# Princic-1837592/julia-raytracer

Hardware: AMD Instinct MI355X
Metric: Mrays/s + wall-clock render time, cornellbox 1280×720×256spp (higher is better)
Workload: dtype f32; 1 GPU; cornellbox path 1280x720x256spp; scene=cornellbox, sampler=path, width=1280, height=720, spp=256, bounces=8, batch=256, traversal=near, traversal_requested=auto, bvh=middle, parallelism=1 tile groups x 1 sample ranges + RCCL reduce

## Files before the change

### julia-raytracer_amd/csrc/jt_kernels.h

```cpp
#pragma once

#include <hip/hip_runtime.h>

#include <algorithm>

#include "jt_bsdf.h"
#include "jt_device.h"
#include "jt_push.h"

#ifndef JT_STAMPS
#define JT_STAMPS 0
#endif
#ifndef JT_NODE_REPEAT_NONE
#define JT_NODE_REPEAT_NONE 4
#endif
#ifndef JT_NODE_REPEAT
#define JT_NODE_REPEAT 3
#endif
#ifndef JT_FIRST_POP_NONE
#define JT_FIRST_POP_NONE 1
#endif
#ifndef JT_FIRST_POP
#define JT_FIRST_POP 2
#endif
// ... 218 lines not shown
    p.scattering = V3(m.scattering[0], m.scattering[1], m.scattering[2]) * xyz(scattering_tex);
    p.scanisotropy = m.scanisotropy;
    p.trdepth = m.trdepth;
    if ((F & FT_VOL) && (mtype == M_REFRACTIVE || mtype == M_VOLUMETRIC || mtype == M_SUBSURFACE)) {
        p.density = V3(-jl_log(jl_clamp(p.color.x, 0.0001f, 1.0f)) / p.trdepth,
                       -jl_log(jl_clamp(p.color.y, 0.0001f, 1.0f)) / p.trdepth,
                       -jl_log(jl_clamp(p.color.z, 0.0001f, 1.0f)) / p.trdepth);
    } else {
        p.density = V3(0, 0, 0);
    }
    if (mtype == M_MATTE || mtype == M_GLTFPBR || mtype == M_GLOSSY) roughness = jl_clamp(roughness, min_roughness, 1.0f);
    else if (mtype == M_VOLUMETRIC) roughness = 0.0f;
    else if (roughness < min_roughness) roughness = 0.0f;
    p.roughness = roughness;
}

template <int F>
__device__ __forceinline__ v3 eval_environment(const DScene& S, v3 direction) {
    v3 emission = V3(0, 0, 0);
    if (!(F & FT_ENV)) return emission;
    for (int k = 0; k < S.nenvs; k++) {
        const DEnv& env = S.envs[k];
        v3 wl = transform_direction(frame_from(env.inv), direction);
        v2 tc = V2(jl_atan2(wl.z, wl.x) / (2.0f * pif), jl_acos(jl_clamp(wl.y, -1.0f, 1.0f)) / pif);
        if (tc.x < 0.0f) tc.x = tc.x + 1.0f;
        v4 t = eval_texture(S, env.tex, tc, false);
        emission = emission + V3(env.emission[0], env.emission[1], env.emission[2]) * xyz(t);
    }
    return emission;
}

constexpr int BLOCK = 256;
constexpr unsigned T_TLAS = 0u, T_INST = 1u, T_BLAS = 2u;
constexpr unsigned IDX_MASK = (1u << 24) - 1;
constexpr unsigned SNAP_NONE = 63u << 24;

struct Hit {
    int inst, elem;
    float u, v, t;
    bool hit;
};
struct Counters {
    unsigned nodes, instances, prims, shades;
};

struct Trav {
    v3 wo, wd, wdinv;
    v3 lo, ld, ldinv;
    float tmax;
    int sp;
    int low;
    int inst_space;
    int negmask;
    int cur_inst, cur_kind;
    int prim, nprim;
    int h_inst, h_elem;
    float h_u, h_v;
    int nh;
    unsigned nxt;
};

#ifndef JT_BAND_STRIP
#define JT_BAND_STRIP 16
#endif
#ifndef JT_TIE_RERUN
#define JT_TIE_RERUN 1
#endif
constexpr int TIE_SEEN = 1 << 8, REF_RERUN = 1 << 9, NH_COUNT = 63;
__device__ __forceinline__ int query_flip(const DScene& S, const Trav& T) { return (T.nh & REF_RERUN) ? 0 : S.order_flip; }
__device__ __forceinline__ void hit_count(Trav& T, float t) {
    T.nh = (T.nh + ((T.nh & NH_COUNT) < NH_COUNT ? 1 : 0)) | (JT_TIE_RERUN && t == T.tmax ? TIE_SEEN : 0);
}

__device__ __forceinline__ int neg_mask(v3 d, int flip) {
    return ((d.x < 0 ? 1 : 0) | (d.y < 0 ? 2 : 0) | (d.z < 0 ? 4 : 0)) ^ flip;
}

__device__ __forceinline__ void world_ray(const DScene& S, Trav& T) {
    T.lo = T.wo;
    T.ld = T.wd;
    T.ldinv = T.wdinv;
    T.negmask = neg_mask(T.wd, query_flip(S, T));
    T.inst_space = 0;
}

__device__ __forceinline__ Hit query_hit(const Trav& T) {
    return Hit{T.h_inst, T.h_elem, T.h_u, T.h_v, T.tmax, T.h_inst >= 0};
}

__device__ __forceinline__ bool query_busy(const Trav& T) { return T.sp > 0 || T.nprim > 0; }
template <bool WIDE>
__device__ __forceinline__ bool wants_node(const Trav& T) {
    return T.nprim == 0 && (T.sp > 0 || (WIDE && T.nxt != W_EMPTY));
}
template <bool WIDE>
__device__ __forceinline__ bool query_done(const Trav& T) {
    return (T.sp | T.nprim) == 0 && (!WIDE || T.nxt == W_EMPTY);
}

__device__ __forceinline__ void query_begin(const DScene& S, Trav& T, v3 o, v3 d, unsigned root, int* stack, int rerun = 0) {
    T.wo = o;
    T.wd = d;
    T.wdinv = V3(jl_rcp(d.x), jl_rcp(d.y), jl_rcp(d.z));
    T.lo = o;
    T.ld = d;
    T.ldinv = T.wdinv;
    T.tmax = __builtin_inff();
    T.nh = rerun;
    T.h_inst = -1;
    T.h_elem = -1;
    T.h_u = 0;
    T.h_v = 0;
    T.nprim = 0;
    T.prim = 0;
    T.cur_inst = -1;
    T.cur_kind = KIND_TRI;
    T.inst_space = 0;
    T.negmask = neg_mask(d, rerun ? 0 : S.order_flip);
    stack[0] = (int)root;
    T.sp = 1;
    T.low = 0;
    T.nxt = W_EMPTY;
}
__device__ __forceinline__ void query_begin_wide(const DScene& S, Trav& T, v3 o, v3 d, unsigned root_word, int rerun = 0) {
    T.wo = o;
    T.wd = d;
    T.wdinv = V3(jl_rcp(d.x), jl_rcp(d.y), jl_rcp(d.z));
    T.lo = o;
    T.ld = d;
    T.ldinv = T.wdinv;
    T.tmax = __builtin_inff();
    T.nh = rerun;
    T.h_inst = -1;
    T.h_elem = -1;
    T.h_u = 0;
    T.h_v = 0;
    T.nprim = 0;
    T.prim = 0;
    T.cur_inst = -1;
    T.cur_kind = KIND_TRI;
    T.inst_space = 0;
    T.negmask = neg_mask(d, rerun ? 0 : S.order_flip);
    T.sp = 0;
    T.low = 0;
    T.nxt = root_word;
}
constexpr unsigned WROOT_SCENE = 0u;
__device__ __forceinline__ unsigned wroot_instance(int inst) { return W_LEAF | W_INST | (unsigned)inst; }
template <bool WIDE>
__device__ __forceinline__ void query_start(const DScene& S, Trav& T, v3 o, v3 d, int inst, int* stack, int rerun = 0) {
    if (WIDE) query_begin_wide(S, T, o, d, inst < 0 ? WROOT_SCENE : wroot_instance(inst), rerun);
    else query_begin(S, T, o, d, inst < 0 ? ((T_TLAS << 30) | SNAP_NONE) : ((T_INST << 30) | SNAP_NONE | (unsigned)inst), stack, rerun);
}
constexpr int INST_LEAF_ROOT = 1 << 30;
template <bool WIDE>
__device__ __forceinline__ bool rerun_tie(const DScene& S, Trav& T, v3 o, v3 d, int inst, int* stack) {
    if (!JT_TIE_RERUN || (T.nh & (TIE_SEEN | REF_RERUN)) != TIE_SEEN || S.order_flip == 0) return false;
    if (inst >= 0 && (S.inst_blas[inst].w & INST_LEAF_ROOT)) return false;
    query_start<WIDE>(S, T, o, d, inst, stack, REF_RERUN);
    return true;
}

template <int F>
__device__ __forceinline__ void tri_pair(const DScene& S, Trav& T, int k) {
    const float4* r = S.prims + 5 * (T.prim + (k >> 1));
    const float4 r0 = r[0], r1 = r[1], r2 = r[2], r3 = r[3], r4 = r[4];
    const PrimHit p1 = intersect_triangle_pre(T.lo, T.ld, ray_eps, V3(r0.x, r0.z, r1.x), V3(r1.z, r2.x, r2.z),
                                              V3(r3.x, r3.z, r4.x));
    const PrimHit p2 = intersect_triangle_pre(T.lo, T.ld, ray_eps, V3(r0.y, r0.w, r1.y), V3(r1.w, r2.y, r2.w),
                                              V3(r3.y, r3.w, r4.y));
    if (tri_hit_before(p1, T.tmax)) {
        hit_count(T, p1.t);
        T.h_inst = T.cur_inst;
        T.h_elem = __float_as_int(r4.z);
        T.h_u = p1.u;
        T.h_v = p1.v;
        T.tmax = p1.t;
    }
    if (T.nprim >= k + 2 && tri_hit_before(p2, T.tmax)) {
        hit_count(T, p2.t);
        T.h_inst = T.cur_inst;
        T.h_elem = __float_as_int(r4.w);
        T.h_u = p2.u;
        T.h_v = p2.v;
        T.tmax = p2.t;
    }
}
template <int COUNT, int F>
__device__ __forceinline__ void prim_step(const DScene& S, Trav& T, Counters& cnt) {
    if (!(F & FT_QUAD) || T.cur_kind == KIND_TRI) {
        tri_pair<F>(S, T, 0);
        const bool more = T.nprim > 2;
        if (__builtin_amdgcn_ballot_w64(more)) {
            if (more) tri_pair<F>(S, T, 2);
        }
        const int n = T.nprim < 4 ? T.nprim : 4;
        if (COUNT) cnt.prims += n;
        T.prim += 2;
        T.nprim -= n;
        return;
    }
    if (COUNT) cnt.prims++;
    const float4* r = S.prims + 4 * T.prim;
    const float4 a = r[0], b = r[1], c = r[2], d = r[3];
    const PrimHit p = intersect_quad(T.lo, T.ld, ray_eps, T.tmax, xyz(a), xyz(b), xyz(c), xyz(d), d.w != 0.0f);
    if (p.hit) {
        hit_count(T, p.t);
        T.h_inst = T.cur_inst;
        T.h_elem = __float_as_int(a.w);
        T.h_u = p.u;
        T.h_v = p.v;
        T.tmax = p.t;
    }
    T.prim += 1;
    T.nprim -= 1;
}

template <int RING, bool OVF>
__device__ __forceinline__ void st_push(const DScene& S, Trav& T, int* stack, int pixel, unsigned e) {
    if (OVF) {
        if (T.sp - T.low == S.ring) {
            S.ovf[(size_t)pixel * S.ovf_stride + T.low] = stack[(T.low & (S.ring - 1)) * BLOCK];
            T.low += 1;
        }
        stack[(T.sp & (S.ring - 1)) * BLOCK] = (int)e;
    } else {
        stack[T.sp * BLOCK] = (int)e;
    }
    T.sp += 1;
}
template <int RING, bool OVF>
__device__ __forceinline__ unsigned st_pop(const DScene& S, Trav& T, const int* stack, int pixel) {
    T.sp -= 1;
    if (OVF) {
        const unsigned r = (unsigned)__hip_atomic_load(stack + (T.sp & (S.ring - 1)) * BLOCK, __ATOMIC_RELAXED,
                                                       __HIP_MEMORY_SCOPE_WORKGROUP);
        if (T.sp < T.low) {
            T.low = T.sp;
            return (unsigned)S.ovf[(size_t)pixel * S.ovf_stride + T.sp];
        }
        return r;
    }
    return (unsigned)stack[T.sp * BLOCK];
}

template <int RING, bool OVF, int COUNT, bool NCACHE, int F>
__device__ __forceinline__ void node_step(const DScene& S, Trav& T, int* stack, int pixel, Counters& cnt) {
    constexpr bool XF = (F & FT_XFORM) != 0;
    const unsigned e = st_pop<RING, OVF>(S, T, stack, pixel);
    unsigned type = e >> 30, idx = e & IDX_MASK;
    if (type == T_INST) {
        if (COUNT) cnt.instances++;
        const int4 ib = S.inst_blas[idx];
        if (!XF || ib.y) {
            if (XF && T.inst_space) world_ray(S, T);
        } else {
            const DInstTrav it = S.inst_trav[idx];
            const fr3 inv = frame_from(it.i0, it.i1, it.i2);
            T.lo = transform_point(inv, T.wo);
            T.ld = transform_vector(inv, T.wd);
            T.ldinv = V3(jl_rcp(T.ld.x), jl_rcp(T.ld.y), jl_rcp(T.ld.z));
            T.negmask = neg_mask(T.ld, query_flip(S, T));
            T.inst_space = 1;
        }
        T.cur_inst = (int)idx;
        T.cur_kind = ib.z;
        type = T_BLAS;
        idx = (unsigned)ib.x;
    } else if (XF && type == T_TLAS && T.inst_space) {
        world_ray(S, T);
    }
    const bool blas = type == T_BLAS;
    if (COUNT) cnt.nodes++;
    const unsigned snap = (e >> 24) & 63u;
    float4 nb;
    if (NCACHE) {
        nb = S.nodes[idx].b;
        __asm__("" : "+v"(nb.x), "+v"(nb.y), "+v"(nb.z), "+v"(nb.w));
        if (snap == 63u || snap != (unsigned)(T.nh & NH_COUNT))
            if (!intersect_bbox(T.lo, T.ldinv, ray_eps, T.tmax, S.nodes[idx].a, nb)) return;
    } else {
        const DNode nd = S.nodes[idx];
        if (!intersect_bbox(T.lo, T.ldinv, ray_eps, T.tmax, nd.a, nd.b)) return;
        nb = nd.b;
    }
    const unsigned meta = __float_as_uint(nb.w);
    const int start = __float_as_int(nb.z);
    const int num = (int)(meta & 0xffffu);
    if (!OVF && !(JT_CHILD_PRETEST && NCACHE)) {
        const PushPlan p = push_plan(meta, start, type, blas, T.negmask, T.sp);
#pragma unroll
        for (int j = 0; j < PUSH_SLOTS; j++) stack[p.slot[j] * BLOCK] = (int)p.value[j];
        T.sp += p.npush;
        T.prim = p.leaf ? start : T.prim;
        T.nprim = p.leaf ? num : T.nprim;
        return;
    }
    if (meta >> 24) {
        const int axis = (int)((meta >> 16) & 0xffu);
        const bool neg = (T.negmask >> axis) & 1;
        const unsigned tag = type << 30 | SNAP_NONE;
        const unsigned c_second = (unsigned)(neg ? start + 1 : start), c_first = (unsigned)(neg ? start : start + 1);
        if (JT_CHILD_PRETEST && NCACHE) {
            const DNode n0 = S.nodes[c_second];
            const DNode n1 = S.nodes[c_first];
            const bool k0 = intersect_bbox(T.lo, T.ldinv, ray_eps, T.tmax, n0.a, n0.b);
// ... 154 lines not shown
        jl_sincos(v * pif, &sv, &cv);
        return transform_direction(frame_from(env.frame), V3(cu * sv, cv, su * sv));
    }
    return V3(0, 0, 0);
}
__device__ __forceinline__ float env_light_pdf(const DScene& S, const DLight l, v3 direction) {
    const float* cdf = S.cdf + l.cdf_offset;
    const DEnv& env = S.envs[l.environment];
    const DTexture t = S.textures[env.tex];
    v3 wl = transform_direction(frame_from(env.inv), direction);
    v2 tc = V2(jl_atan2(wl.z, wl.x) / (2 * pif), jl_acos(jl_clamp(wl.y, -1.0f, 1.0f)) / pif);
    if (tc.x < 0) tc.x = tc.x + 1;
    int i = jl_clampi((int)__builtin_truncf(tc.x * (float)t.width), 0, t.width - 1);
    int j = jl_clampi((int)__builtin_truncf(tc.y * (float)t.height), 0, t.height - 1);
    float prob = sample_discrete_pdf(cdf, j * t.width + i + 1) / cdf[l.ncdf - 1];
    float angle = (2 * pif / (float)t.width) * (pif / (float)t.height) *
                  jl_sin(pif * ((float)j + 0.5f) / (float)t.height);
    return prob / angle;
}

enum : int { PH_SCENE = 0, PH_LIGHT = 1, PH_FINISH = 2 };
__host__ __device__ constexpr bool light_steps(int sampler, int F) {
    return sampler == 1 && !(F & FT_ENV) && !(F & FT_LINL);
}
__device__ __forceinline__ bool chains_inline(int F, const DScene& S) { return !(F & FT_NOIL) && ((F & FT_LINL) || S.light_inline); }
enum : int { F_HIT = 1, F_VOLUME = 2 };

constexpr unsigned CTL_BOUNCE = 0x7fffu, CTL_OPB = 15, CTL_FLAGS = 23, CTL_LC = 25;
#ifndef JT_PARK
#define JT_PARK 1
#endif
#ifndef JT_PARK_PB
#define JT_PARK_PB 1
#endif
constexpr int PARK_SLOTS = 7 + (JT_PARK_PB ? 1 : 0);
__host__ __device__ constexpr bool park(int F) { return JT_PARK != 0 && !ft_none(F); }
__host__ __device__ constexpr bool park_lq(int F) { return park(F); }
__host__ __device__ constexpr int park_slots(int F) { return park(F) ? PARK_SLOTS : 0; }
struct Path {
    v3 o, d;
    v3 radiance_, weight_;
    Rng rng;
    unsigned ctl;
    int phase;
    float max_roughness_;
    float* pk;
    int li;
    template <int F>
    __device__ __forceinline__ v3 radiance() const {
        return park(F) ? V3(pk[0], pk[BLOCK], pk[2 * BLOCK]) : radiance_;
    }
    template <int F>
    __device__ __forceinline__ void set_radiance(v3 v) {
        if (park(F)) {
            pk[0] = v.x;
            pk[BLOCK] = v.y;
            pk[2 * BLOCK] = v.z;
        } else {
            radiance_ = v;
        }
    }
    template <int F>
    __device__ __forceinline__ v3 lq() const { return park_lq(F) ? V3(pk[4 * BLOCK], pk[5 * BLOCK], pk[6 * BLOCK]) : lq_; }
    template <int F>
    __device__ __forceinline__ void set_lq(v3 v) {
        if (park_lq(F)) {
            pk[4 * BLOCK] = v.x;
            pk[5 * BLOCK] = v.y;
            pk[6 * BLOCK] = v.z;
        } else {
            lq_ = v;
        }
    }
    template <int F>
    __device__ __forceinline__ float max_roughness() const { return park(F) ? pk[3 * BLOCK] : max_roughness_; }
    template <int F>
    __device__ __forceinline__ void set_max_roughness(float v) {
        if (park(F)) pk[3 * BLOCK] = v;
        else max_roughness_ = v;
    }
    template <int F>
    __device__ __forceinline__ float pb() const { return park(F) && JT_PARK_PB ? pk[7 * BLOCK] : pb_; }
    template <int F>
    __device__ __forceinline__ void set_pb(float v) {
        if (park(F) && JT_PARK_PB) pk[7 * BLOCK] = v;
        else pb_ = v;
    }
    template <int F>
    __device__ __forceinline__ v3 weight() const { return weight_; }
    template <int F>
    __device__ __forceinline__ void set_weight(v3 v) { weight_ = v; }
    __device__ __forceinline__ int bounce() const { return (int)(ctl & CTL_BOUNCE); }
    __device__ __forceinline__ int opbounce() const { return (int)((ctl >> CTL_OPB) & 0xffu); }
    __device__ __forceinline__ bool flag(int f) const { return (ctl >> CTL_FLAGS) & (unsigned)f; }
    __device__ __forceinline__ void set_flag(int f) { ctl |= (unsigned)f << CTL_FLAGS; }
    __device__ __forceinline__ void clear_flag(int f) { ctl &= ~((unsigned)f << CTL_FLAGS); }
    __device__ __forceinline__ int lcount() const { return (int)(ctl >> CTL_LC); }
    v3 lq_;
    float pb_;
    float pdf, lpdf;
    Volume vol;
};

__device__ __forceinline__ bool next_bounce(const DParams& P, Path& st) {
    if (st.bounce() >= P.bounces) return true;
    st.ctl += 1u;
    st.phase = PH_SCENE;
    return false;
}
__device__ __forceinline__ bool next_bounce_retry(const DParams& P, Path& st) {
    if (st.bounce() - 1 >= P.bounces) return true;
    st.phase = PH_SCENE;
    return false;
}
template <int F>
__device__ __forceinline__ bool after_weight(const DParams& P, Path& st) {
    if (is_zero(st.weight<F>()) || !all_finite(st.weight<F>())) return true;
    if (st.bounce() > 3) {
        float rr_prob = jl_min(0.99f, max3(st.weight<F>()));
        if (rand1f(st.rng) >= rr_prob) return true;
        st.set_weight<F>(st.weight<F>() * (1 / rr_prob));
    }
    return next_bounce(P, st);
}
template <int F>
__device__ __forceinline__ bool light_advance(const DScene& S, const DParams& P, Path& st) {
    for (;;) {
        st.li += 1;
        if (st.li >= S.nlights) {
            st.o = st.lq<F>();
            const float pdf = st.pdf * S.light_pick_pdf;
            st.set_weight<F>(st.weight<F>() / (0.5f * st.pb<F>() + 0.5f * pdf));
            return after_weight<F>(P, st);
        }
        const DLight l = S.lights[st.li];
        if (!(F & FT_NOIL) && l.instance >= 0) {
            st.lpdf = 0.0f;
            st.ctl &= (1u << CTL_LC) - 1u;
            st.o = st.lq<F>();
            st.phase = PH_LIGHT;
            return false;
        }
        if ((F & FT_ENV) && l.environment >= 0) st.pdf += env_light_pdf(S, l, st.d);
    }
}
template <int F>
__device__ __forceinline__ bool begin_light_pdf(const DScene& S, const DParams& P, Path& st) {
    st.pdf = 0.0f;
    st.li = -1;
    st.set_lq<F>(st.o);
    return light_advance<F>(S, P, st);
}
template <int F>
__device__ __forceinline__ bool light_hit(const DScene& S, const DParams& P, Path& st, const Hit& h) {
    if (h.hit) {
        const int4 lh = row16<F>(S.light_hit + st.li);
        const DInstShade& is = S.inst_shade[lh.x];
        const fr3 f = frame_from(is.f0, is.f1, is.f2);
        const float4* r = S.light_elems + 5 * (lh.y + h.elem);
        const float4 r0 = r[0], r1 = r[1], r2 = r[2], r3 = r[3];
        const v3 p1 = V3(r0.x, r0.y, r0.z), p2 = V3(r0.w, r1.x, r1.y), p3 = V3(r1.z, r1.w, r2.x);
        const v2 uv = V2(h.u, h.v);
        v3 lposition;
        if (!(F & FT_QUAD) || __float_as_int(r3.z) == KIND_TRI) {
            lposition = transform_point(f, interp_tri(p1, p2, p3, uv));
        } else {
            const float4 r4 = r[4];
            lposition = transform_point(f, interp_quad(p1, p2, p3, V3(r4.x, r4.y, r4.z), uv));
        }
        const v3 en = V3(r2.y, r2.z, r2.w);
        v3 lnormal = __float_as_int(r3.y) ? en : transform_normal(f, en);
        const float area = r3.x;
        v3 dd = lposition - st.lq<F>();
        st.lpdf += dot(dd, dd) / (__builtin_fabsf(dot(lnormal, st.d)) * area);
        st.o = lposition + st.d * 0.001f;
        st.ctl += 1u << CTL_LC;
        if (st.lcount() < 100) return false;
    }
    st.pdf += st.lpdf;
    return light_advance<F>(S, P, st);
}

#ifndef JT_LIGHT_LEAF_STEP
#define JT_LIGHT_LEAF_STEP 1
#endif
template <int COUNT, int F>
__device__ __forceinline__ void inst_leaf_query(const DScene& S, Trav& T, v3 o, v3 d, v3 dinv, int negmask, int inst,
                                                Counters& cnt) {
    constexpr bool XF = (F & FT_XFORM) != 0;
    T.wo = o;
    T.wd = d;
    T.wdinv = dinv;
    T.lo = o;
    T.ld = d;
    T.ldinv = dinv;
    T.tmax = __builtin_inff();
    T.nh = 0;
    T.h_inst = -1;
    T.h_elem = -1;
    T.h_u = 0;
    T.h_v = 0;
    T.inst_space = 0;
    T.negmask = negmask;
    T.sp = 0;
    T.low = 0;
    T.nxt = W_EMPTY;
    if (COUNT) cnt.instances++;
    const int4 ib = S.inst_blas[inst];
    if (XF && !ib.y) {
        const DInstTrav it = S.inst_trav[inst];
        const fr3 inv = frame_from(it.i0, it.i1, it.i2);
        T.lo = transform_point(inv, T.wo);
        T.ld = transform_vector(inv, T.wd);
        T.ldinv = V3(jl_rcp(T.ld.x), jl_rcp(T.ld.y), jl_rcp(T.ld.z));
        T.negmask = neg_mask(T.ld, query_flip(S, T));
        T.inst_space = 1;
    }
    T.cur_inst = inst;
    T.cur_kind = ib.z;
    if (COUNT) cnt.nodes++;
    const DNode nd = S.nodes[ib.x];
    const bool pass = intersect_bbox(T.lo, T.ldinv, ray_eps, T.tmax, nd.a, nd.b);
    T.prim = pass ? __float_as_int(nd.b.z) : 0;
    T.nprim = pass ? (int)(__float_as_uint(nd.b.w) & 0xffffu) : 0;
}

template <bool WIDE, int RING, bool OVF, int COUNT, bool NCACHE, int F, class CountLq>
__device__ __forceinline__ bool light_chain(const DScene& S, const DParams& P, Path& st, Trav& T, int* stack, int pixel,
                                            Counters& cnt, CountLq count_lq) {
    constexpr bool RERUN_LOOP = (F & ~FT_LINL) == (FT_TEX | FT_ATTR | FT_MAT | FT_OPAC | FT_XFORM);
    if (JT_LIGHT_LEAF_STEP && !WIDE && !OVF && !NCACHE && !RERUN_LOOP) {
        do {
            count_lq();
            const v3 d = st.d;
            const v3 dinv = V3(jl_rcp(d.x), jl_rcp(d.y), jl_rcp(d.z));
            const int negmask = neg_mask(d, S.order_flip);
            inst_leaf_query<COUNT, F>(S, T, st.o, d, dinv, negmask, S.lights[st.li].instance, cnt);
            while (T.nprim > 0) prim_step<COUNT, F>(S, T, cnt);
            if (light_hit<F>(S, P, st, query_hit(T))) return true;
        } while (st.phase == PH_LIGHT);
        return false;
    }
    do {
        count_lq();
        const int inst = S.lights[st.li].instance;
        query_start<WIDE>(S, T, st.o, st.d, inst, stack);
        do {
            node_step_any<WIDE, RING, OVF, COUNT, NCACHE, F>(S, T, stack, pixel, cnt);
            while (T.nprim > 0) prim_step<COUNT, F>(S, T, cnt);
        } while (RERUN_LOOP && rerun_tie<WIDE>(S, T, st.o, st.d, inst, stack));
        if (light_hit<F>(S, P, st, query_hit(T))) return true;
    } while (st.phase == PH_LIGHT);
    return false;
}

#ifndef JT_LANE_LDS
#define JT_LANE_LDS 1
#endif
#ifndef JT_LANE_LDS_NONE
#define JT_LANE_LDS_NONE 1
#endif
__host__ __device__ constexpr bool lane_lds(int F) { return JT_LANE_LDS && (!ft_none(F) || JT_LANE_LDS_NONE); }
constexpr int ACC_SLOTS = (JT_LANE_LDS ? 13 : 11) + (JT_PARK ? PARK_SLOTS : 0);
__host__ __device__ constexpr int acc_base_slots(int F) { return lane_lds(F) ? (ft_none(F) ? 12 : 13) : 11; }
__host__ __device__ constexpr int acc_slots(int F) { return acc_base_slots(F) + park_slots(F); }
struct Aov {
    float* acc;
    float w_;
    int first_;
    int lk_;
    template <int F>
    __device__ __forceinline__ float w() const {
        if (!lane_lds(F)) return w_;
        if (ft_none(F)) return 1.0f / (float)(((reinterpret_cast<const int*>(acc)[11 * BLOCK] - first_) >> lk_) + 1);
        return acc[12 * BLOCK];
    }
};
template <int F>
__device__ __forceinline__ void aov_update(const Aov& a, v3 ta, v3 tn) {
    const float aw = a.w<F>();
    const float omw = 1 - aw;
    float* p = a.acc;
    p[4 * BLOCK] = p[4 * BLOCK] * omw + ta.x * aw;
    p[5 * BLOCK] = p[5 * BLOCK] * omw + ta.y * aw;
    p[6 * BLOCK] = p[6 * BLOCK] * omw + ta.z * aw;
    p[7 * BLOCK] = p[7 * BLOCK] * omw + tn.x * aw;
    p[8 * BLOCK] = p[8 * BLOCK] * omw + tn.y * aw;
    p[9 * BLOCK] = p[9 * BLOCK] * omw + tn.z * aw;
}

template <int F, class AovT>
__device__ __forceinline__ bool path_hit(const DScene& S, const DParams& P, Path& st, Hit isec, const AovT& aov,
                                         unsigned& shades) {
    if (!isec.hit) {
        if (st.bounce() > 0 || !P.envhidden)
            st.set_radiance<F>(st.radiance<F>() + st.weight<F>() * eval_environment<F>(S, st.d));
        return true;
    }
    bool in_volume = false;
    if ((F & FT_VOL) && st.flag(F_VOLUME)) {
        float rl = rand1f(st.rng), rd = rand1f(st.rng);
        float distance = sample_transmittance(st.vol.density, isec.t, rl, rd);
        v3 tr = eval_transmittance(st.vol.density, distance);
        float tp = sample_transmittance_pdf(st.vol.density, distance, isec.t);
        st.set_weight<F>((st.weight<F>() * tr) / tp);
        in_volume = distance < isec.t;
        isec.t = distance;
    }
    if (!in_volume) {
        v3 outgoing = -st.d;
        Shading sh;
        eval_shading<F>(S, isec.inst, isec.elem, V2(isec.u, isec.v), outgoing, sh);
        shades++;
        if (P.nocaustics) {
            st.set_max_roughness<F>(jl_max(sh.mat.roughness, st.max_roughness<F>()));
            sh.mat.roughness = st.max_roughness<F>();
        }
        if ((F & FT_OPAC) && sh.mat.opacity < 1 && rand1f(st.rng) >= sh.mat.opacity) {
            if (st.opbounce() > 128) return true;
            st.ctl += 1u << CTL_OPB;
            st.o = sh.position + st.d * 0.01f;
            return next_bounce_retry(P, st);
        }
        if (st.bounce() == 0) {
            st.set_flag(F_HIT);
            aov_update<F>(aov, sh.mat.color, sh.normal);
        }
        st.set_radiance<F>(st.radiance<F>() + st.weight<F>() * (dot(sh.normal, outgoing) >= 0 ? sh.mat.emission : V3(0, 0, 0)));
        v3 incoming;
        const bool delta = is_delta(sh.mat);
        if (!delta) {
            if (rand1f(st.rng) < 0.5f) {
                float rnl = rand1f(st.rng);
                v2 rn = rand2f(st.rng);
                incoming = sample_bsdfcos<F>(sh.mat, sh.normal, outgoing, rnl, rn);
            } else {
                float rl = rand1f(st.rng), rel = rand1f(st.rng);
                v2 ruv = rand2f(st.rng);
                incoming = sample_lights<F>(S, sh.position, rl, rel, ruv);
            }
            if (is_zero(incoming)) return true;
#if JT_FUSED_BSDF
            v3 fb;
            float pbv;
            eval_bsdfcos_pdf<F>(sh.mat, sh.normal, outgoing, incoming, fb, pbv);
            st.set_weight<F>(st.weight<F>() * fb);
            st.set_pb<F>(pbv);
#else
            st.set_weight<F>(st.weight<F>() * eval_bsdfcos<F>(sh.mat, sh.normal, outgoing, incoming));
            st.set_pb<F>(sample_bsdfcos_pdf<F>(sh.mat, sh.normal, outgoing, incoming));
#endif
        } else {
            float rnl = rand1f(st.rng);
            incoming = sample_delta<F>(sh.mat, sh.normal, outgoing, rnl);
            v3 f = eval_delta<F>(sh.mat, sh.normal, outgoing, incoming);
            float pd = sample_delta_pdf<F>(sh.mat, sh.normal, outgoing, incoming);
            st.set_weight<F>((st.weight<F>() * f) / pd);
        }
        const int mtype = sh.mat.type;
        if ((F & FT_VOL) && (mtype == M_REFRACTIVE || mtype == M_VOLUMETRIC || mtype == M_SUBSURFACE) &&
            dot(sh.normal, outgoing) * dot(sh.normal, incoming) < 0) {
            if (!st.flag(F_VOLUME)) {
                st.set_flag(F_VOLUME);
                st.vol.density = sh.mat.density;
                st.vol.scattering = sh.mat.scattering;
                st.vol.scanisotropy = sh.mat.scanisotropy;
            } else {
                st.clear_flag(F_VOLUME);
            }
        }
        st.o = sh.position;
        st.d = incoming;
        return delta ? after_weight<F>(P, st) : begin_light_pdf<F>(S, P, st);
    }
    v3 outgoing = -st.d;
    v3 position = st.o + st.d * isec.t;
    v3 incoming;
    if (rand1f(st.rng) < 0.5f) {
        (void)rand1f(st.rng);
        v2 rn = rand2f(st.rng);
        incoming = sample_scattering(st.vol, outgoing, rn);
    } else {
        float rl = rand1f(st.rng), rel = rand1f(st.rng);
        v2 ruv = rand2f(st.rng);
        incoming = sample_lights<F>(S, position, rl, rel, ruv);
    }
    if (is_zero(incoming)) return true;
    st.set_weight<F>(st.weight<F>() * eval_scattering(st.vol, outgoing, incoming));
    st.set_pb<F>(sample_scattering_pdf(st.vol, outgoing, incoming));
    st.o = position;
    st.d = incoming;
    return begin_light_pdf<F>(S, P, st);
}

template <int F, class AovT>
__device__ __forceinline__ bool naive_hit(const DScene& S, const DParams& P, Path& st, Hit isec, const AovT& aov,
                                          unsigned& shades) {
    if (!isec.hit) {
        if (st.bounce() > 0 || !P.envhidden)
            st.set_radiance<F>(st.radiance<F>() + st.weight<F>() * eval_environment<F>(S, st.d));
        return true;
    }
    v3 outgoing = -st.d;
// ... 312 lines not shown
                            im = JT_A(image)[pixel];
                            al = JT_A(albedo)[pixel];
                            nr = JT_A(normal)[pixel];
                            h = (int)JT_A(hits)[pixel];
                        } else {
                            const size_t o = (size_t)((s - P.first) & (kstr - 1)) * (size_t)JT_A(nslot) +
                                             (size_t)item_slot(item, P);
                            im = JT_A(part_img)[o];
                            al = JT_A(part_alb)[o];
                            nr = JT_A(part_nrm)[o];
                            h = __float_as_int(al.w);
                        }
                    }
                    acc[0] = im.x;
                    acc[BLOCK] = im.y;
                    acc[2 * BLOCK] = im.z;
                    acc[3 * BLOCK] = im.w;
                    acc[4 * BLOCK] = al.x;
                    acc[5 * BLOCK] = al.y;
                    acc[6 * BLOCK] = al.z;
                    acc[7 * BLOCK] = nr.x;
                    acc[8 * BLOCK] = nr.y;
                    acc[9 * BLOCK] = nr.z;
                    acc_i[10 * BLOCK] = h;
                }
            }
            bnext += take;
        }
        next_sample = false;
        if (start) {
            const int sample = acc_i[11 * BLOCK];
            const int pixel = item_pixel(item, P, tiles_x);
            if (!ft_none(F)) acc[12 * BLOCK] = stream_weight(P, sample);
            const DParams& P = karg_params<karg_params_on<SAMPLER, F>()>(P0);
            start_path<F>(P, pixel % P.width, pixel / P.width, pixel, sample, st);
            query_start<WIDE>(S, T, st.o, st.d, -1, stack);
            if (!WC) lds_count(1, true);
            if constexpr (item_first_pop<WIDE, F>()) {
#pragma unroll
                for (int k = 0; k < (!ft_none(F) && (F & FT_LINL) ? JT_FIRST_POP : JT_FIRST_POP_NONE); k++)
                    if (wants_node<WIDE>(T)) node_step_any<WIDE, RING, OVF, COUNT, NCACHE, F>(S, T, stack, oslot, cnt);
            }
        }
        if (WC) w_rays += lane_count(__builtin_amdgcn_ballot_w64(start));
#if JT_STAMPS
        const unsigned long long ts1 = __builtin_amdgcn_s_memtime();
        t_start += ts1 - ts0;
        n_start++;
        lanes_start += lane_count(__builtin_amdgcn_ballot_w64(start));
#endif
        if (__builtin_amdgcn_ballot_w64(item != ITEM_NONE) == 0) break;
        constexpr bool LSTEP = light_steps(SAMPLER, F);
        for (;;) {
            const bool wantp = T.nprim > 0;
            const bool wantn = wants_node<WIDE>(T);
            const bool waiting = query_done<WIDE>(T);
            const int np = lane_count(__builtin_amdgcn_ballot_w64(wantp));
            const int nn = lane_count(__builtin_amdgcn_ballot_w64(wantn));
            int nw = lane_count(__builtin_amdgcn_ballot_w64(waiting));
            const int nb = np + nn;
            if (LSTEP && !S.light_inline) {
                const bool wantl = waiting && st.phase == PH_LIGHT;
                const int nl = lane_count(__builtin_amdgcn_ballot_w64(wantl));
                if (nl > 0 && (nl >= P.light_lanes || nb == 0)) {
                    bool c_lq = false, c_ray = false;
                    if (wantl && rerun_tie<WIDE>(S, T, st.o, st.d, S.lights[st.li].instance, stack)) {
                    } else if (wantl) {
                        if (light_hit<F>(S, P, st, query_hit(T))) {
                            st.phase = PH_FINISH;
                        } else if (st.phase == PH_LIGHT) {
                            if (WC) c_lq = true;
                            else lds_count(2, true);
                            query_start<WIDE>(S, T, st.o, st.d, S.lights[st.li].instance, stack);
                        } else {
                            if (WC) c_ray = true;
                            else lds_count(1, true);
                            query_start<WIDE>(S, T, st.o, st.d, -1, stack);
                        }
                    }
                    if (WC) {
                        w_lq += lane_count(__builtin_amdgcn_ballot_w64(c_lq));
                        w_rays += lane_count(__builtin_amdgcn_ballot_w64(c_ray));
                    }
                    continue;
                }
                nw -= nl;
            }
            if (nb == 0 || nw >= (nb + nw < P.wait_lanes ? nb + nw : P.wait_lanes)) break;
#if JT_STAMPS
            n_trav++;
            idle += 64 - lane_count(__builtin_amdgcn_ballot_w64(item != ITEM_NONE));
            if (np * JT_VOTE_P >= nn * JT_VOTE_N) { steps_p++; lanes_p += np; } else { steps_n++; lanes_n += nn; }
#endif
            if (JT_RAY_FROM_PATH && !(F & FT_XFORM)) {
                T.lo = st.o;
                T.ld = st.d;
            }
            if (np * JT_VOTE_P >= nn * JT_VOTE_N) {
                if (T.nprim > 0) prim_step<COUNT, F>(S, T, cnt);
            } else {
                constexpr int NREP = ft_none(F) ? JT_NODE_REPEAT_NONE : JT_NODE_REPEAT;
#pragma unroll
                for (int k = 0; k < NREP; k++)
                    if (wants_node<WIDE>(T)) node_step_any<WIDE, RING, OVF, COUNT, NCACHE, F>(S, T, stack, oslot, cnt);
            }
        }
#if JT_STAMPS
        const unsigned long long ts2 = __builtin_amdgcn_s_memtime();
        t_trav += ts2 - ts1;
        n_shade++;
        lanes_sh += lane_count(__builtin_amdgcn_ballot_w64(query_done<WIDE>(T)));
        {
            int mid = -1, mt = -1;
            if (query_done<WIDE>(T) && st.phase == PH_SCENE && T.h_inst >= 0) {
                mid = S.inst_shade[T.h_inst].material;
                mt = (F & FT_MAT) ? S.materials[mid].type : (int)M_MATTE;
            }
            if (__builtin_amdgcn_ballot_w64(mt >= 0)) {
                n_mph++;
                lanes_hit += lane_count(__builtin_amdgcn_ballot_w64(mt >= 0));
                for (int ty = 0; ty <= (int)M_GLTFPBR; ty++) n_mty += __builtin_amdgcn_ballot_w64(mt == ty) ? 1u : 0u;
                bool counted = mt < 0;
                for (;;) {
                    const unsigned long long m = __builtin_amdgcn_ballot_w64(!counted);
                    if (!m) break;
                    const int v = __shfl(mid, __ffsll((long long)m) - 1);
                    counted = counted || mid == v;
                    n_mid++;
                }
            }
        }
        unsigned long long ts3 = ts2, ts4 = ts2;
#endif
        constexpr bool LINL = (F & (FT_LINL | FT_NOIL)) != 0;
        {
            const bool tie = query_done<WIDE>(T) && (T.nh & (TIE_SEEN | REF_RERUN)) == TIE_SEEN &&
                             !(LSTEP && st.phase == PH_FINISH);
            if (S.order_flip && __builtin_amdgcn_ballot_w64(tie))
                if (tie) rerun_tie<WIDE>(S, T, st.o, st.d, SAMPLER == 1 && !LINL && st.phase == PH_LIGHT ? S.lights[st.li].instance : -1, stack);
        }
        bool c_path = false, c_lq = false, c_ray = false;
        unsigned n_inl = 0;
        if (query_done<WIDE>(T)) {
            const DParams& P = karg_params<karg_params_on<SAMPLER, F>()>(P0);
            const DScene SL = shade_scene_lds<NCACHE, RING, OVF, F>(S0);
            const DScene& S = NCACHE ? shade_scene<karg_scene<NCACHE, F>()>(S0) : SL;
            bool alive = true;
            const bool light = SAMPLER == 1 && !LINL && st.phase == PH_LIGHT;
            bool done;
            if (LSTEP && st.phase == PH_FINISH) done = true;
            else if (light) done = light_hit<F>(S, P, st, query_hit(T));
            else if (SAMPLER == 2) done = naive_hit<F>(S, P, st, query_hit(T), aov, cnt.shades);
            else done = path_hit<F>(S, P, st, query_hit(T), aov, cnt.shades);
            if (SAMPLER == 1 && !done && st.phase == PH_LIGHT && chains_inline(F, S)) {
                unsigned nlq = 0;
                done = light_chain<WIDE, RING, OVF, COUNT, NCACHE, F>(S, P, st, T, stack, oslot, cnt, [&] {
                    if (WC) nlq++;
                    else lds_count(2, true);
                });
                if (WC) n_inl += nlq;
            }
#if JT_STAMPS
            ts3 = __builtin_amdgcn_s_memtime();
            n_phit++;
#endif
            if (done) {
                if (WC) c_path = true;
                else lds_count(0, true);
                v3 radiance = st.radiance<F>();
                if (!all_finite(radiance)) radiance = V3(0, 0, 0);
                const float mr = max3(radiance);
                if (mr > P.clamp) radiance = radiance * (P.clamp / mr);
                const float w = aov.w<F>();
                const float omw = 1 - w;
                const bool hit = st.flag(F_HIT);
                const bool env = !hit && !P.envhidden && S.nenvs != 0;
                const v4 target = (hit || env) ? V4(radiance.x, radiance.y, radiance.z, 1) : V4(0, 0, 0, 0);
                if (!hit) aov_update<F>(aov, env ? V3(1, 1, 1) : V3(0, 0, 0), -st.d);
                acc[0] = acc[0] * omw + target.x * w;
                acc[BLOCK] = acc[BLOCK] * omw + target.y * w;
                acc[2 * BLOCK] = acc[2 * BLOCK] * omw + target.z * w;
                acc[3 * BLOCK] = acc[3 * BLOCK] * omw + target.w * w;
                if (hit || env) acc_i[10 * BLOCK] += 1;
                alive = false;
                T.sp = -1;
                const int sample = acc_i[11 * BLOCK];
                if (sample + kstr >= JT_SE) {
                    const int pixel = item_pixel(item, P, tiles_x);
                    const float4 im = make_float4(acc[0], acc[BLOCK], acc[2 * BLOCK], acc[3 * BLOCK]);
                    if (P.lk == 0) {
                        JT_A(image)[pixel] = im;
                        JT_A(albedo)[pixel] = make_float4(acc[4 * BLOCK], acc[5 * BLOCK], acc[6 * BLOCK], 0.0f);
                        JT_A(normal)[pixel] = make_float4(acc[7 * BLOCK], acc[8 * BLOCK], acc[9 * BLOCK], 0.0f);
                        JT_A(hits)[pixel] = (long long)acc_i[10 * BLOCK];
                    } else {
                        const size_t o = (size_t)((sample - P.first) & (kstr - 1)) * (size_t)JT_A(nslot) +
                                         (size_t)item_slot(item, P);
                        JT_A(part_img)[o] = im;
                        JT_A(part_alb)[o] = make_float4(acc[4 * BLOCK], acc[5 * BLOCK], acc[6 * BLOCK], __int_as_float(acc_i[10 * BLOCK]));
                        JT_A(part_nrm)[o] = make_float4(acc[7 * BLOCK], acc[8 * BLOCK], acc[9 * BLOCK], 0.0f);
                    }
                    item = ITEM_NONE;
                } else {
                    acc_i[11 * BLOCK] = sample + kstr;
                    next_sample = true;
                }
            }
#if JT_STAMPS
            ts4 = __builtin_amdgcn_s_memtime();
            if (__builtin_amdgcn_ballot_w64(done)) n_fin++;
#endif
            if (alive) {
                if (SAMPLER == 1 && !LINL && st.phase == PH_LIGHT) {
                    if (WC) c_lq = true;
                    else lds_count(2, true);
                    query_start<WIDE>(S, T, st.o, st.d, S.lights[st.li].instance, stack);
                } else {
                    if (WC) c_ray = true;
                    else lds_count(1, true);
                    query_start<WIDE>(S, T, st.o, st.d, -1, stack);
                }
#pragma unroll
                for (int k = 0; k < (!ft_none(F) && (F & FT_LINL) ? JT_FIRST_POP : JT_FIRST_POP_NONE); k++)
                    if (wants_node<WIDE>(T)) node_step_any<WIDE, RING, OVF, COUNT, NCACHE, F>(S, T, stack, oslot, cnt);
            }
        }
#if JT_STAMPS
        const unsigned long long ts5 = __builtin_amdgcn_s_memtime();
        t_shade += ts5 - ts2;
        t_hit += ts3 - ts2;
        t_fin += ts4 - ts3;
        t_qb += ts5 - ts4;
#endif
        if (WC) {
            w_paths += lane_count(__builtin_amdgcn_ballot_w64(c_path));
            w_lq += lane_count(__builtin_amdgcn_ballot_w64(c_lq));
            w_rays += lane_count(__builtin_amdgcn_ballot_w64(c_ray));
            if (SAMPLER == 1 && chains_inline(F, S)) w_lq += __builtin_amdgcn_readfirstlane(wave_sum(n_inl));
        }
    }
#if JT_STAMPS
    if (lane == 0) {
        unsigned long long* dbg = A.counters + 8;
        const unsigned long long v[24] = {t_trav, t_shade, n_trav,  n_shade, lanes_p, lanes_n,  steps_p, steps_n,
                                          0,      t_hit,   t_fin,   t_qb,    0,       n_phit,   n_fin,   idle,
                                          n_mph,  n_mty,   n_mid,   lanes_sh, lanes_hit, t_start, n_start, lanes_start};
        for (int k = 0; k < 24; k++) atomicAdd(dbg + k, v[k]);
    }
#endif
    const unsigned wv[3] = {w_paths, w_rays, w_lq};
    unsigned v[7] = {0u, 0u, 0u, cnt.nodes, cnt.instances, cnt.prims, COUNT ? cnt.shades : 0u};
#pragma unroll
    for (int k = 0; k < 7; k++) {
        unsigned sum = k < 3 ? (WC ? wv[k] : wcnt[k]) : wave_sum(v[k]);
        if (lane == 0 && sum) atomicAdd(&A.counters[k], (unsigned long long)sum);
    }
}

struct DCombine {
    float w[JT_MAX_STREAMS];
    int ns;
};
inline void combine_weights(long long n, int lk, DCombine& cw) {
    cw = DCombine{};
    cw.ns = combine_weights(n, lk, cw.w);
}
#ifndef JT_WAVES
#define JT_WAVES 0
#endif
#ifndef JT_WAVES_NONE
#define JT_WAVES_NONE 5
#endif
#if JT_WAVES > 0
#define JT_WAVES_PER_EU __attribute__((amdgpu_waves_per_eu(JT_WAVES, JT_WAVES)))
#define JT_WAVES_PER_EU_F(F) \
    __attribute__((amdgpu_waves_per_eu(ft_none(F) ? JT_WAVES_NONE : JT_WAVES, ft_none(F) ? JT_WAVES_NONE : JT_WAVES)))
#else
#define JT_WAVES_PER_EU
#define JT_WAVES_PER_EU_F(F)
#endif
__host__ __device__ constexpr size_t lds_stack_bytes(bool ovf, int ring, int need) {
    return (size_t)(ovf ? ring : need) * BLOCK * 4;
}

__device__ __forceinline__ DScene blob_scene(const DScene& S, const uint4* blob) {
    DScene L = S;
    L.nodes = reinterpret_cast<const DNode*>(blob + S.o_nodes);
    L.wnodes = reinterpret_cast<const DWide*>(blob + S.o_wnodes);
    L.prims = reinterpret_cast<const float4*>(blob + S.o_prims);
    L.inst_trav = reinterpret_cast<const DInstTrav*>(blob + S.o_inst_trav);
    L.inst_blas = reinterpret_cast<const int4*>(blob + S.o_inst_blas);
    L.inst_shade = reinterpret_cast<const DInstShade*>(blob + S.o_inst_shade);
    L.shapes = reinterpret_cast<const DShape*>(blob + S.o_shapes);
    L.pos = reinterpret_cast<const float4*>(blob + S.o_pos);
    L.nrm = reinterpret_cast<const float4*>(blob + S.o_nrm);
    L.tc = reinterpret_cast<const float2*>(blob + S.o_tc);
    L.col = reinterpret_cast<const float4*>(blob + S.o_col);
    L.elems = reinterpret_cast<const int4*>(blob + S.o_elems);
    L.enrm = reinterpret_cast<const float4*>(blob + S.o_enrm);
    L.enrm_id = reinterpret_cast<const float4*>(blob + S.o_enrm_id);
    L.materials = reinterpret_cast<const DMaterial*>(blob + S.o_materials);
    L.lights = reinterpret_cast<const DLight*>(blob + S.o_lights);
    L.light_hit = reinterpret_cast<const int4*>(blob + S.o_light_hit);
    L.light_elems = reinterpret_cast<const float4*>(blob + S.o_light_elems);
    L.cdf = reinterpret_cast<const float*>(blob + S.o_cdf);
    return L;
}

template <int SAMPLER, int RING, bool OVF, int COUNT, int F, bool WIDE>
__global__ __launch_bounds__(BLOCK) JT_WAVES_PER_EU void trace_kernel(DScene S, DParams P, int s_begin, int s_end, DAccum A) {
    __shared__ int lds_stack[RING * BLOCK];
    trace_body_items<SAMPLER, RING, OVF, COUNT, F, true, WIDE>(S, P, s_begin, s_end, A, lds_stack + threadIdx.x);
}

template <int SAMPLER, int RING, bool OVF, int COUNT, int F, bool WIDE>
__global__ __launch_bounds__(BLOCK) JT_WAVES_PER_EU_F(F) void trace_kernel_lds(DScene S, DParams P, int s_begin, int s_end, DAccum A) {
    extern __shared__ uint4 dyn_lds[];
    uint4* blob = dyn_lds + lds_stack_bytes(OVF, RING, S.stack_need) / 16;
    for (int k = threadIdx.x; k < S.blob_n16; k += BLOCK) blob[k] = S.blob[k];
    __syncthreads();
    const DScene L = blob_scene(S, blob);
    trace_body_items<SAMPLER, RING, OVF, COUNT, F, false, WIDE>(L, P, s_begin, s_end, A, reinterpret_cast<int*>(dyn_lds) + threadIdx.x);
}

template <int SAMPLER, int RING, bool OVF, int COUNT, int F, bool LDSK, bool WIDE>
hipError_t launch_t(const DScene& S, const DParams& P, int s0, int s1, const DAccum& A, hipStream_t st, int cus) {
    const long long units = (long long)launch_tiles(P) * std::min(s1 - s0, 1 << P.lk);
    const int want = (int)std::min<long long>((units + BLOCK / 64 - 1) / (BLOCK / 64), 1 << 30);
    if (want == 0) return hipSuccess;
    int per_cu = 0;
    hipError_t e;
    if constexpr (LDSK) {
        if (S.blob_n16 > 0) {
        const size_t lds = lds_stack_bytes(OVF, RING, S.stack_need) + (size_t)S.blob_n16 * 16;
        const void* k = (const void*)trace_kernel_lds<SAMPLER, RING, OVF, COUNT, F, WIDE>;
        if ((e = hipFuncSetAttribute(k, hipFuncAttributeMaxDynamicSharedMemorySize, (int)lds)) != hipSuccess) return e;
        if (hipOccupancyMaxActiveBlocksPerMultiprocessor(&per_cu, k, BLOCK, lds) != hipSuccess || per_cu < 1) per_cu = 1;
        const int nwg = std::min(want, std::min(per_cu, 8) * cus);
        hipLaunchKernelGGL((trace_kernel_lds<SAMPLER, RING, OVF, COUNT, F, WIDE>), dim3(nwg), dim3(BLOCK), lds, st, S, P, s0, s1, A);
        return hipGetLastError();
        }
    }
    const void* k = (const void*)trace_kernel<SAMPLER, RING, OVF, COUNT, F, WIDE>;
    if (hipOccupancyMaxActiveBlocksPerMultiprocessor(&per_cu, k, BLOCK, 0) != hipSuccess || per_cu < 1) per_cu = 1;
    const int nwg = std::min(want, std::min(per_cu, 8) * cus);
    hipLaunchKernelGGL((trace_kernel<SAMPLER, RING, OVF, COUNT, F, WIDE>), dim3(nwg), dim3(BLOCK), 0, st, S, P, s0, s1, A);
    return hipGetLastError();
}

constexpr int FT_MESH = FT_TEX | FT_ATTR | FT_MAT | FT_OPAC | FT_XFORM;
constexpr int FT_MESH_ENV = FT_MESH | FT_ENV;
constexpr int FT_MESH_ENV_QUAD = FT_MESH_ENV | FT_QUAD;
inline int kernel_mask(int feat, int need, int ring, bool lds, bool linl, bool inst_light) {
    if (need <= 16) return feat == FT_NONE ? (linl ? FT_NONE | FT_LINL : FT_NONE) : FT_ALL;
    if (ring > 16 || lds) return FT_ALL;
    for (int m : {FT_MESH | FT_LINL, FT_MESH_ENV | FT_NOIL, FT_MESH_ENV_QUAD | FT_LINL})
        if (!(feat & ~m & ~(FT_LINL | FT_NOIL)) && ((m & FT_LINL) ? linl : !inst_light)) return m;
    return FT_ALL;
}

constexpr int NUM_BASE_CONFIGS = 8;
template <int ID>
struct LaunchConfig;
#define JT_LAUNCH_CONFIG(ID, R, O, F, L)                            \
    template <>                                                      \
    struct LaunchConfig<ID> {                                        \
        static constexpr int ring = R;                               \
        static constexpr bool ovf = O;                               \
        static constexpr int feat = F;                               \
        static constexpr bool lds = L;                               \
        static constexpr bool wide = false;                          \
    };                                                               \
    template <>                                                      \
// ... 27 lines not shown
```

Baseline: 12070 Mrays/s.

## Restructure inline light chain to compute ray reciprocal once and reuse it on restart

Splits light_hit into an accumulate step and a chain-end step so the inline light chain can loop over repeated instance-leaf queries without re-entering the full advance logic on each hit. When the tail path applies, the ray direction reciprocal and negmask are computed once per chain and kept in the traversal state. A new query_restart then reuses that reciprocal for the next scene ray when the whole wave took the chained path, skipping the usual query_begin setup. This adds a wave ballot, more template branching, and a reliance on T.wdinv staying valid for the next ray's direction.

```diff
diff --git a/julia-raytracer_amd/csrc/jt_kernels.h b/julia-raytracer_amd/csrc/jt_kernels.h
--- a/julia-raytracer_amd/csrc/jt_kernels.h
+++ b/julia-raytracer_amd/csrc/jt_kernels.h
@@ -394,6 +394,30 @@
     if (WIDE) query_begin_wide(S, T, o, d, inst < 0 ? WROOT_SCENE : wroot_instance(inst), rerun);
     else query_begin(S, T, o, d, inst < 0 ? ((T_TLAS << 30) | SNAP_NONE) : ((T_INST << 30) | SNAP_NONE | (unsigned)inst), stack, rerun);
 }
+template <int F>
+__device__ __forceinline__ void query_restart(const DScene& S, Trav& T, v3 o, v3 d, int* stack) {
+    T.wo = o;
+    T.wd = d;
+    T.lo = o;
+    T.ld = d;
+    T.ldinv = T.wdinv;
+    T.tmax = __builtin_inff();
+    T.nh = 0;
+    T.h_inst = -1;
+    T.h_elem = -1;
+    T.h_u = 0;
+    T.h_v = 0;
+    T.nprim = 0;
+    T.prim = 0;
+    T.cur_inst = -1;
+    T.cur_kind = KIND_TRI;
+    T.inst_space = 0;
+    if (F & FT_XFORM) T.negmask = neg_mask(d, S.order_flip);
+    stack[0] = (int)((T_TLAS << 30) | SNAP_NONE);
+    T.sp = 1;
+    T.low = 0;
+    T.nxt = W_EMPTY;
+}
 constexpr int INST_LEAF_ROOT = 1 << 30;
 template <bool WIDE>
 __device__ __forceinline__ bool rerun_tie(const DScene& S, Trav& T, v3 o, v3 d, int inst, int* stack) {
@@ -854,38 +878,62 @@
     return light_advance<F>(S, P, st);
 }
 template <int F>
-__device__ __forceinline__ bool light_hit(const DScene& S, const DParams& P, Path& st, const Hit& h) {
-    if (h.hit) {
-        const int4 lh = row16<F>(S.light_hit + st.li);
-        const DInstShade& is = S.inst_shade[lh.x];
-        const fr3 f = frame_from(is.f0, is.f1, is.f2);
-        const float4* r = S.light_elems + 5 * (lh.y + h.elem);
-        const float4 r0 = r[0], r1 = r[1], r2 = r[2], r3 = r[3];
-        const v3 p1 = V3(r0.x, r0.y, r0.z), p2 = V3(r0.w, r1.x, r1.y), p3 = V3(r1.z, r1.w, r2.x);
-        const v2 uv = V2(h.u, h.v);
-        v3 lposition;
-        if (!(F & FT_QUAD) || __float_as_int(r3.z) == KIND_TRI) {
-            lposition = transform_point(f, interp_tri(p1, p2, p3, uv));
-        } else {
-            const float4 r4 = r[4];
-            lposition = transform_point(f, interp_quad(p1, p2, p3, V3(r4.x, r4.y, r4.z), uv));
-        }
-        const v3 en = V3(r2.y, r2.z, r2.w);
-        v3 lnormal = __float_as_int(r3.y) ? en : transform_normal(f, en);
-        const float area = r3.x;
-        v3 dd = lposition - st.lq<F>();
-        st.lpdf += dot(dd, dd) / (__builtin_fabsf(dot(lnormal, st.d)) * area);
-        st.o = lposition + st.d * 0.001f;
-        st.ctl += 1u << CTL_LC;
-        if (st.lcount() < 100) return false;
-    }
+__device__ __forceinline__ bool light_hit_add(const DScene& S, Path& st, const Hit& h) {
+    const int4 lh = row16<F>(S.light_hit + st.li);
+    const DInstShade& is = S.inst_shade[lh.x];
+    const fr3 f = frame_from(is.f0, is.f1, is.f2);
+    const float4* r = S.light_elems + 5 * (lh.y + h.elem);
+    const float4 r0 = r[0], r1 = r[1], r2 = r[2], r3 = r[3];
+    const v3 p1 = V3(r0.x, r0.y, r0.z), p2 = V3(r0.w, r1.x, r1.y), p3 = V3(r1.z, r1.w, r2.x);
+    const v2 uv = V2(h.u, h.v);
+    v3 lposition;
+    if (!(F & FT_QUAD) || __float_as_int(r3.z) == KIND_TRI) {
+        lposition = transform_point(f, interp_tri(p1, p2, p3, uv));
+    } else {
+        const float4 r4 = r[4];
+        lposition = transform_point(f, interp_quad(p1, p2, p3, V3(r4.x, r4.y, r4.z), uv));
+    }
+    const v3 en = V3(r2.y, r2.z, r2.w);
+    v3 lnormal = __float_as_int(r3.y) ? en : transform_normal(f, en);
+    const float area = r3.x;
+    v3 dd = lposition - st.lq<F>();
+    st.lpdf += dot(dd, dd) / (__builtin_fabsf(dot(lnormal, st.d)) * area);
+    st.o = lposition + st.d * 0.001f;
+    st.ctl += 1u << CTL_LC;
+    return st.lcount() < 100;
+}
+template <int F>
+__device__ __forceinline__ bool light_chain_end(const DScene& S, const DParams& P, Path& st) {
     st.pdf += st.lpdf;
     return light_advance<F>(S, P, st);
 }
+template <int F>
+__device__ __forceinline__ bool light_hit(const DScene& S, const DParams& P, Path& st, const Hit& h) {
+    if (h.hit && light_hit_add<F>(S, st, h)) return false;
+    return light_chain_end<F>(S, P, st);
+}
 
 #ifndef JT_LIGHT_LEAF_STEP
 #define JT_LIGHT_LEAF_STEP 1
 #endif
+#ifndef JT_CHAIN_TAIL
+#define JT_CHAIN_TAIL 2
+#endif
+__host__ __device__ constexpr bool ft_mesh_kernel(int F) {
+    return (F & ~FT_LINL) == (FT_TEX | FT_ATTR | FT_MAT | FT_OPAC | FT_XFORM);
+}
+template <bool WIDE, int F>
+__host__ __device__ constexpr bool chain_tail() {
+    return JT_CHAIN_TAIL && !WIDE && !(F & FT_NOIL) && F != FT_NONE && !ft_mesh_kernel(F);
+}
+template <bool WIDE, bool OVF, bool NCACHE, int F>
+__host__ __device__ constexpr bool chain_leaf_step() {
+    return JT_LIGHT_LEAF_STEP && !WIDE && !OVF && !NCACHE && !ft_mesh_kernel(F);
+}
+template <bool WIDE, bool OVF, bool NCACHE, int F>
+__host__ __device__ constexpr bool chain_dinv_once() {
+    return JT_CHAIN_TAIL >= 2 && chain_tail<WIDE, F>() && chain_leaf_step<WIDE, OVF, NCACHE, F>();
+}
 template <int COUNT, int F>
 __device__ __forceinline__ void inst_leaf_query(const DScene& S, Trav& T, v3 o, v3 d, v3 dinv, int negmask, int inst,
                                                 Counters& cnt) {
@@ -930,27 +978,40 @@
 template <bool WIDE, int RING, bool OVF, int COUNT, bool NCACHE, int F, class CountLq>
 __device__ __forceinline__ bool light_chain(const DScene& S, const DParams& P, Path& st, Trav& T, int* stack, int pixel,
                                             Counters& cnt, CountLq count_lq) {
-    constexpr bool RERUN_LOOP = (F & ~FT_LINL) == (FT_TEX | FT_ATTR | FT_MAT | FT_OPAC | FT_XFORM);
-    if (JT_LIGHT_LEAF_STEP && !WIDE && !OVF && !NCACHE && !RERUN_LOOP) {
-        do {
-            count_lq();
-            const v3 d = st.d;
-            const v3 dinv = V3(jl_rcp(d.x), jl_rcp(d.y), jl_rcp(d.z));
-            const int negmask = neg_mask(d, S.order_flip);
-            inst_leaf_query<COUNT, F>(S, T, st.o, d, dinv, negmask, S.lights[st.li].instance, cnt);
-            while (T.nprim > 0) prim_step<COUNT, F>(S, T, cnt);
-            if (light_hit<F>(S, P, st, query_hit(T))) return true;
-        } while (st.phase == PH_LIGHT);
-        return false;
-    }
-    do {
+    constexpr bool RERUN_LOOP = ft_mesh_kernel(F);
+    constexpr bool LEAF = chain_leaf_step<WIDE, OVF, NCACHE, F>(), TAIL = chain_tail<WIDE, F>();
+    constexpr bool DINV_ONCE = chain_dinv_once<WIDE, OVF, NCACHE, F>();
+    const auto dinv = [&] { T.wdinv = V3(jl_rcp(st.d.x), jl_rcp(st.d.y), jl_rcp(st.d.z)); };
+    const auto query = [&] {
         count_lq();
         const int inst = S.lights[st.li].instance;
-        query_start<WIDE>(S, T, st.o, st.d, inst, stack);
-        do {
-            node_step_any<WIDE, RING, OVF, COUNT, NCACHE, F>(S, T, stack, pixel, cnt);
+        if (LEAF) {
+            if (!DINV_ONCE) dinv();
+            const int negmask = DINV_ONCE && !(F & FT_XFORM) ? T.negmask : neg_mask(st.d, S.order_flip);
+            inst_leaf_query<COUNT, F>(S, T, st.o, st.d, T.wdinv, negmask, inst, cnt);
             while (T.nprim > 0) prim_step<COUNT, F>(S, T, cnt);
-        } while (RERUN_LOOP && rerun_tie<WIDE>(S, T, st.o, st.d, inst, stack));
+        } else {
+            query_start<WIDE>(S, T, st.o, st.d, inst, stack);
+            do {
+                node_step_any<WIDE, RING, OVF, COUNT, NCACHE, F>(S, T, stack, pixel, cnt);
+                while (T.nprim > 0) prim_step<COUNT, F>(S, T, cnt);
+            } while (RERUN_LOOP && rerun_tie<WIDE>(S, T, st.o, st.d, inst, stack));
+        }
+    };
+    if (TAIL) {
+        if (DINV_ONCE) {
+            dinv();
+            if (!(F & FT_XFORM)) T.negmask = neg_mask(st.d, S.order_flip);
+        }
+        for (;;) {
+            do query();
+            while (T.h_inst >= 0 && light_hit_add<F>(S, st, query_hit(T)));
+            if (light_chain_end<F>(S, P, st)) return true;
+            if (st.phase != PH_LIGHT) return false;
+        }
+    }
+    do {
+        query();
         if (light_hit<F>(S, P, st, query_hit(T))) return true;
     } while (st.phase == PH_LIGHT);
     return false;
@@ -1569,8 +1630,10 @@
             else if (light) done = light_hit<F>(S, P, st, query_hit(T));
             else if (SAMPLER == 2) done = naive_hit<F>(S, P, st, query_hit(T), aov, cnt.shades);
             else done = path_hit<F>(S, P, st, query_hit(T), aov, cnt.shades);
+            bool chained = false;
             if (SAMPLER == 1 && !done && st.phase == PH_LIGHT && chains_inline(F, S)) {
                 unsigned nlq = 0;
+                chained = true;
                 done = light_chain<WIDE, RING, OVF, COUNT, NCACHE, F>(S, P, st, T, stack, oslot, cnt, [&] {
                     if (WC) nlq++;
                     else lds_count(2, true);
@@ -1635,7 +1698,9 @@
                 } else {
                     if (WC) c_ray = true;
                     else lds_count(1, true);
-                    query_start<WIDE>(S, T, st.o, st.d, -1, stack);
+                    if (SAMPLER == 1 && chain_dinv_once<WIDE, OVF, NCACHE, F>() && __builtin_amdgcn_ballot_w64(!chained) == 0)
+                        query_restart<F>(S, T, st.o, st.d, stack);
+                    else query_start<WIDE>(S, T, st.o, st.d, -1, stack);
                 }
 #pragma unroll
                 for (int k = 0; k < (!ft_none(F) && (F & FT_LINL) ? JT_FIRST_POP : JT_FIRST_POP_NONE); k++)
```

After: 12530 Mrays/s, median of 6. 3.8% higher.
